# bee-hive/MedGP

Hardware: AMD Instinct MI355X
Metric: per-patient nlml+grad evals/sec at D=24 N=512 (higher is better)
Workload: dtype f64; 1 GPU; config 4 shard: 512 patients/GPU x N=512, D=24, Q=5, R=8, H=1114, LMC-SM + hier-gamma prior, nlml+grad; patients_per_gpu=512, cohort=512, N=512, D=24, Q=5, R=8, H=1114, parallelism=patient-sharded x1 (no collective)

## Files before the change

medgp_amd/csrc/call_plan.h:

```cpp
#pragma once
#include <algorithm>
#include <cstddef>
#include <vector>

#ifndef MEDGP_HD
#if defined(__HIPCC__) || defined(__HIP__)
#define MEDGP_HD __host__ __device__
#else
#define MEDGP_HD
#endif
#endif

#define LA_SLICE 4
MEDGP_HD inline int la_slice_len(int k) { return k < 32 ? LA_SLICE : (k < 44 ? LA_SLICE + 1 : LA_SLICE + 2); }

struct PlanRules {
    int Q = 0, D = 0;
    int num_cu = 256;
    int max_batch = 0;
    size_t mem_budget = (size_t)64 << 30;
    size_t screen_budget = (size_t)2 << 30;
    long long screen_work = 32768;
    int screen_lanes = 2;
    int no_classes = 0;
// ... 25 lines not shown
    int row0 = 0;
    size_t mat0 = 0, vec0 = 0, tab0 = 0, la_part0 = 0, la_small0 = 0;
};

inline int tri(int n) { return n * (n + 1) / 2; }
inline int blocks64(int n) { return (std::max(n, 1) + 63) / 64; }
inline int size_bucket(int nb) { int j = 0; while ((1 << j) < nb) j++; return j; }
inline long long wg_cost(int nb) { return (long long)nb * nb * (nb + 17); }

struct WgradGrid { bool ragged; int nbp, wg_tiles; int grid; };
inline WgradGrid wgrad_grid(const int *entry_n, int nbatch, int nt64) {
    WgradGrid g{false, nbatch, tri(nt64), 0};
    for (int bb = 1; bb < nbatch; bb++) g.ragged = g.ragged || blocks64(entry_n[bb]) != blocks64(entry_n[0]);
    if (g.ragged && nbatch < 64) g.nbp = nbatch | 1;
    g.grid = std::max(8 * ((nbatch + 7) / 8), g.nbp) * g.wg_tiles;
    return g;
}

struct SlabGeom { int R, C; size_t stride; };
inline SlabGeom slab_geom(int ld, int Q, int D) {
    SlabGeom g{ld / 16 + D, ld / 64 + D, 0};
    g.stride = (size_t)3 * Q * g.R * g.C;
    return g;
}

inline void layout_plan(const PlanRules &r, const int *en, int nbatch, bool with_u, BatchPlan &P) {
    P.order.resize(nbatch); P.inv.resize(nbatch); P.en.resize(nbatch);
    P.cls.clear();
    P.with_u = with_u;
    int mx = 0;
    for (int b = 0; b < nbatch; b++) { P.order[b] = b; mx = std::max(mx, en[b]); }
    const bool classes = !r.no_classes;
    if (classes) std::stable_sort(P.order.begin(), P.order.end(), [&](int a, int b) { return blocks64(en[a]) > blocks64(en[b]); });
    P.identity = true;
    for (int i = 0; i < nbatch; i++) { P.inv[P.order[i]] = i; P.en[i] = en[P.order[i]]; P.identity = P.identity && P.order[i] == i; }
    const size_t Q = r.Q, bpe = with_u ? 16 : 8;
    size_t om = 0, ov = 0, ot = 0, os = 0, wave_bytes = 0;
    int wave = 0;
    P.need_mat = P.need_vec = P.need_tab = P.need_slab = 0;
    for (int i = 0; i < nbatch;) {
        SizeClass k;
        k.b0 = i;
        const int bk = size_bucket(blocks64(P.en[i]));
        k.nbmax = classes ? blocks64(P.en[i]) : blocks64(mx);
        k.ld = 64 * k.nbmax;
        const size_t per = bpe * (size_t)k.ld * k.ld;
// ... 133 lines not shown
```

medgp_amd/csrc/kernels_core.h:

```cpp
#pragma once
#include "medgp_dev.h"

#define PREP_CHUNK 2048
#define PREP_BCHUNK 256
__device__ __forceinline__ double prep_w(const MedgpDev &L, const double *th, int q) {
    if (L.kidx == 7) return 2.0 * L.pi * exp(th[L.D + L.Q * L.D * L.R + q]);
    if (L.kidx == 8) return 2.0 * L.pi * exp(th[1 + L.Q + q]);
    return 0.0;
}
__global__ void __launch_bounds__(256) k_prep(MedgpDev L, const double *__restrict__ theta, int min_n) {
    const int b = blockIdx.x, tid = threadIdx.x, nt = blockDim.x;
    const int slot = L.bslot[b];
    const int n = L.pn[slot];
    const double *th = theta + (size_t)(L.tpos ? L.tpos[b] : (L.bpos ? L.bpos[b] : b)) * L.H;
    double *hyp = L.hyp + (size_t)b * L.hyp_stride;
    double *sig2 = hyp, *B = hyp + hyp_off_B(L), *w = hyp + hyp_off_w(L), *c = hyp + hyp_off_c(L);
    const int Q = L.Q, D = L.D, R = L.R;
    const double pi = L.pi;
    const int ntab = (Q * L.ldn + PREP_CHUNK - 1) / PREP_CHUNK;
    if ((int)blockIdx.y > ntab) {
        if (theta == nullptr || L.kidx != 7) return;
        const int idx = ((int)blockIdx.y - ntab - 1) * PREP_BCHUNK + tid;
        if (idx >= Q * D * D) return;
        const double *A = th + D, *lk = th + D + Q * (D * R + 2);
// ... 83 lines not shown
    const int ld = L.ldn;
    const double *hyp = L.hyp + (size_t)b * L.hyp_stride;
    const double *cs = L.cs + (size_t)b * L.Q * ld, *sn = L.sn + (size_t)b * L.Q * ld;
    const double *t = L.pt + (size_t)slot * L.pld;
    const int *meta = L.pmeta + (size_t)slot * L.pld;
    double *K = L.Kmat + (size_t)b * ld * ld;
    for (int idx = threadIdx.x; idx < np * np; idx += blockDim.x) {
        int i = idx / np, j = idx - i * np;
        if (j > i) continue;
        double v;
        if (i < n && j < n) {
            v = cov_elem(L, hyp, cs, sn, t, meta, i, j);
            if (i == j) {
                double lik = hyp[meta[i]];
                v += lik;
                for (int r = 0; r < count; r++) v += lik;
            }
        } else v = (i == j) ? 1.0 : 0.0;
        K[(size_t)i * ld + j] = v;
    }
    __syncthreads();
}

__global__ void __launch_bounds__(256) k_slabsum(MedgpDev L) {
    __shared__ int s_roff[MEDGP_MAX_D + 1], s_coff[MEDGP_MAX_D + 1], s_seg[MEDGP_MAX_D + 1];
    const int b = blockIdx.x, tid = threadIdx.x, nt = blockDim.x;
    if (L.status[b] < 0) return;
    const int Q = L.Q, D = L.D;
    const int slot = L.bslot[b];
    for (int i = tid; i <= D; i += nt) {
        s_roff[i] = L.proff[(size_t)slot * (D + 1) + i];
        s_coff[i] = L.pcoff[(size_t)slot * (D + 1) + i];
        s_seg[i] = L.pseg[(size_t)slot * (D + 1) + i];
    }
    __syncthreads();
    const int *roff = s_roff, *coff = s_coff, *seg = s_seg;
    const double *slab = L.slab + (size_t)b * L.slab_stride;
    const int nbins = D * (D + 1) / 2;
    const int idx = blockIdx.y * nt + tid;
    if (idx >= 3 * Q * nbins) return;
    const int pq = idx / nbins;
    int d, e;
    tile_decode(idx - pq * nbins, d, e);
    const double *sl = slab + (size_t)pq * L.slab_R * L.slab_C;
    double s = 0.0;
    for (int rs = roff[d]; rs < roff[d + 1]; rs++) {
        const int It = (seg[d] / 16 + (rs - roff[d])) / 4;
        for (int cs = coff[e]; cs < coff[e + 1]; cs++) {
            const int Jt = seg[e] / 64 + (cs - coff[e]);
            if (Jt <= It) s += sl[(size_t)rs * L.slab_C + cs];
        }
    }
    const int pl = pq / Q, q = pq - pl * Q;
    double *dst = (pl == 0 ? L.S : (pl == 1 ? L.SM : L.SV)) + (size_t)b * Q * D * D;
    dst[(size_t)q * D * D + d * D + e] = s;
}

__device__ inline void prior_apply(const MedgpPrior &p, double hv, double pi, bool want_grad, double &lp_sum, double &g) {
    if (!p.flag) return;
    if (p.type == 0) { if (want_grad) g = 0.0; return; }
    double lp, dlp;
    if (p.type == 1) {
        lp = -1.0 * (hv - p.p0) * (hv - p.p0) / (2.0 * p.p1);
        lp = lp - log(2 * pi * p.p1) / 2.0;
        dlp = -1.0 * (hv - p.p0) / p.p1;
    } else if (p.type == 2) {
        lp = (-1.0 * fabs(hv - p.p0) / p.p1) - (double)p.lg2b;
        if (hv == p.p0) dlp = 0.0;
        else dlp = -1.0 * ((hv > p.p0) ? 1.0 : -1.0) / p.p1;
    } else return;
    lp_sum += lp;
    if (want_grad) g -= p.is_exp ? hv * dlp : dlp;
}

__device__ inline double sym_get(const double *S, int D, int d, int e) { return d >= e ? S[d * D + e] : S[e * D + d]; }

__global__ void __launch_bounds__(256) k_epilogue(MedgpDev L, const double *__restrict__ theta, int flag_grad, int from_slab,
                                                  double *__restrict__ nlml_out, double *__restrict__ grad_out,
                                                  int *__restrict__ status_out, int loo_objective = 0) {
    __shared__ double red2[MEDGP_EPI_PARTS][256];
    constexpr int EPI_S_MAX = 4096, EPI_A_MAX = 1280;
    __shared__ double s_S[EPI_S_MAX], s_A[EPI_A_MAX];
    const int b = blockIdx.x, tid = threadIdx.x, nt = blockDim.x;
    const int H = L.H, Q = L.Q, D = L.D, R = L.R, ld = L.ldn;
    const int part = blockIdx.y, nparts = gridDim.y;
    const int nchunk = min(MEDGP_EPI_PARTS, (H + 255) / 256), hchunk = (H + nchunk - 1) / nchunk;
    const int cpp = (nchunk + nparts - 1) / nparts, ch0 = part * cpp, ch1 = min(nchunk, ch0 + cpp);
    const int h0 = ch0 * hchunk, h1 = min(H, ch1 * hchunk);
    const int hA0 = L.kidx == 7 ? D : H, hA1 = L.kidx == 7 ? D + Q * D * R : H, hMV1 = L.kidx == 7 ? D + Q * (D * R + 2) : H;
    const bool own_A = h0 < hA1 && h1 > hA0, own_muv = h0 < hMV1 && h1 > hA1;
    const bool lds_sa = flag_grad && L.kidx == 7 && own_A && Q * D * D <= EPI_S_MAX && Q * D * R <= EPI_A_MAX;
    const int st = L.status[b];
    const int pos = L.bpos ? L.bpos[b] : b;
    double *g = grad_out ? grad_out + (size_t)pos * H : nullptr;
    if (tid == 0 && part == 0 && status_out) status_out[pos] = st;
    if (st < 0) {
        if (tid == 0 && part == 0 && loo_objective != 2) nlml_out[pos] = __builtin_nan("");
        if (flag_grad && g) for (int h = h0 + tid; h < h1; h += nt) g[h] = __builtin_nan("");
        return;
    }
    const int slot = L.bslot[b], n = L.pn[slot];
    const double *th = theta + (size_t)(L.tpos ? L.tpos[b] : pos) * H;
    const double *hyp = L.hyp + (size_t)b * L.hyp_stride;
    const double *B = hyp + hyp_off_B(L);
    const double *S = L.S + (size_t)b * Q * D * D, *SM = L.SM + (size_t)b * Q * D * D, *SV = L.SV + (size_t)b * Q * D * D;
    const int *seg = L.pseg + (size_t)slot * (D + 1);
    const double *Wd = from_slab ? L.wdiag + (size_t)b * ld : L.Kmat + (size_t)b * ld * ld;
    const size_t wds = from_slab ? 1 : (size_t)ld + 1;
    if (lds_sa) {
        for (int i = tid; i < Q * D * D; i += nt) s_S[i] = S[i];
        for (int i = tid; i < Q * D * R; i += nt) s_A[i] = th[D + i];
        __syncthreads();
    }
    __shared__ double smuv[64];
    const bool par_muv = flag_grad && L.kidx == 7 && own_muv && 2 * Q <= 64;
    if (par_muv) {
        const int nbins = D * (D + 1) / 2, lane = tid & 63, nwave = nt >> 6;
        for (int w2 = tid >> 6; w2 < 2 * Q; w2 += nwave) {
            const int q = (w2 < Q) ? w2 : w2 - Q;
            const double *X = ((w2 < Q) ? SM : SV) + (size_t)q * D * D, *Bq = B + (size_t)q * D * D;
            double sacc = 0.0;
            int d, e;
            tile_decode(lane, d, e);
            for (int idx = lane; idx < nbins; idx += 64) {
                sacc += ((d == e) ? 1.0 : 2.0) * Bq[d * D + e] * X[d * D + e];
                e += 64;
                while (e > d) { e -= d + 1; d++; }
            }
            for (int off = 32; off > 0; off >>= 1) sacc += __shfl_xor(sacc, off);
            if (lane == 0) smuv[w2] = sacc;
        }
        __syncthreads();
    }
    __shared__ double s_sig[MEDGP_MAX_D];
    const bool par_sig = flag_grad && L.kidx == 7 && h0 < D;
    if (par_sig) {
        const int lane = tid & 63, nwave = nt >> 6, dhi = min(D, h1);
        for (int d = h0 + (tid >> 6); d < dhi; d += nwave) {
            double sacc = 0.0;
            for (int i = seg[d] + lane; i < seg[d + 1]; i += 64) sacc += Wd[(size_t)i * wds];
            for (int off = 32; off > 0; off >>= 1) sacc += __shfl_xor(sacc, off);
            if (lane == 0) s_sig[d] = sacc;
        }
        __syncthreads();
    }
    const int pslot = slot >= L.max_slots ? slot - L.max_slots : slot;
    const MedgpPrior *pr = (loo_objective != 2 && L.prior_on[pslot]) ? L.prior + (size_t)pslot * H : nullptr;
    double lp_part = 0.0;
  for (int ch = ch0; ch < ch1; ch++) {
    double lp_local = 0.0;
    const int hc1 = min(H, (ch + 1) * hchunk);
    for (int h = ch * hchunk + tid; h < hc1; h += nt) {
        double gv = 0.0, hv;
        if (L.kidx == 7) {
            if (h < D) {
                hv = exp(th[h]);
                if (flag_grad) gv = (hv * hv) * s_sig[h];
            } else {
                int hc = h - D;
                if (hc < Q * D * R) {
                    hv = th[h];
                    if (flag_grad) {
                        int q = hc / (D * R), rem = hc - q * D * R, d = rem / R, r = rem - d * R;
                        double s = 0.0;
                        if (lds_sa) {
                            const double *A = s_A + q * D * R, *Sq = s_S + q * D * D;
                            for (int e = 0; e < D; e++) s += sym_get(Sq, D, d, e) * A[e * R + r];
                        } else {
                            const double *A = th + D + (size_t)q * D * R;
                            const double *Sq = S + (size_t)q * D * D;
                            int e = 0;
                            for (; e + 8 <= D; e += 8) {
                                double sv[8], av[8];
#pragma unroll
                                for (int u = 0; u < 8; u++) {
                                    const int ee = e + u, ix = (d >= ee) ? d * D + ee : ee * D + d;
                                    sv[u] = Sq[ix];
                                    av[u] = A[ee * R + r];
                                }
#pragma unroll
                                for (int u = 0; u < 8; u++) s += sv[u] * av[u];
                            }
                            for (; e < D; e++) s += sym_get(Sq, D, d, e) * A[e * R + r];
                        }
                        gv = s;
                    }
                } else if (hc < Q * (D * R + 2)) {
                    hv = exp(th[h]);
                    if (flag_grad) {
                        bool is_mu = hc < Q * (D * R + 1);
                        int q = is_mu ? hc - Q * D * R : hc - Q * (D * R + 1);
                        if (par_muv) gv = 0.5 * smuv[is_mu ? q : Q + q];
                        else {
                            const double *X = (is_mu ? SM : SV) + (size_t)q * D * D, *Bq = B + (size_t)q * D * D;
                            double s = 0.0;
                            for (int d = 0; d < D; d++)
                                for (int e = 0; e <= d; e++) s += ((d == e) ? 1.0 : 2.0) * Bq[d * D + e] * X[d * D + e];
                            gv = 0.5 * s;
                        }
                    }
                } else {
                    hv = exp(th[h]);
                    if (flag_grad) {
                        int kk = hc - Q * (D * R + 2), q = kk / D, d = kk - q * D;
                        gv = 0.5 * hv * S[(size_t)q * D * D + d * D + d];
                    }
                }
            }
        } else if (L.kidx == 8) {
            hv = exp(th[h]);
            if (flag_grad) {
                if (h == 0) {
                    double s = 0.0;
                    for (int i = 0; i < n; i++) s += hv * hv * Wd[(size_t)i * wds];
                    gv = s;
                } else {
                    int hc = h - 1, mode = hc / Q, q = hc - mode * Q;
                    const double *X = mode == 0 ? S : (mode == 1 ? SM : SV);
                    gv = 0.5 * B[q] * X[q];
                }
            }
        } else {
            hv = exp(th[h]);
            if (flag_grad) {
                if (h == 0) {
                    double s = 0.0;
                    for (int i = 0; i < n; i++) s += hv * hv * Wd[(size_t)i * wds];
                    gv = s;
                } else if (h == 1) gv = -0.5 * B[0] * SV[0];
                else gv = B[0] * S[0];
            }
        }
        if (pr) prior_apply(pr[h], hv, L.pi, flag_grad != 0, lp_local, gv);
        if (flag_grad && g) g[h] = gv;
    }
    red2[ch - ch0][tid] = lp_local;
  }
    {
        const int nc = ch1 - ch0;
        __syncthreads();
        for (int off = 128; off > 0; off >>= 1) {
            if (tid < off)
                for (int c2 = 0; c2 < nc; c2++) red2[c2][tid] += red2[c2][tid + off];
            __syncthreads();
        }
        if (tid == 0)
            for (int c2 = 0; c2 < nc; c2++) {
                if (nparts > 1) __hip_atomic_store(&L.epi_lp[(size_t)b * MEDGP_EPI_PARTS + ch0 + c2], red2[c2][0], __ATOMIC_RELAXED, __HIP_MEMORY_SCOPE_AGENT);
                lp_part += red2[c2][0];
            }
    }
    if (tid == 0) {
        double lp = lp_part;
        if (nparts > 1) {
            __threadfence();
            const int ticket = __hip_atomic_fetch_add(&L.epi_ticket[b], 1, __ATOMIC_ACQ_REL, __HIP_MEMORY_SCOPE_AGENT);
            if (ticket != nparts - 1) return;
            __threadfence();
            lp = 0.0;
            for (int c2 = 0; c2 < nchunk; c2++)
                lp += __hip_atomic_load(&L.epi_lp[(size_t)b * MEDGP_EPI_PARTS + c2], __ATOMIC_RELAXED, __HIP_MEMORY_SCOPE_AGENT);
            __hip_atomic_store(&L.epi_ticket[b], 0, __ATOMIC_RELAXED, __HIP_MEMORY_SCOPE_AGENT);
        }
        double logdet = L.scal[b * 4 + 0], quad = L.scal[b * 4 + 1];
        double nlml = quad / 2.0 + logdet + n * log(2. * L.pi) / 2.0;
        if (loo_objective) nlml = L.scal[b * 4 + 2];
        if (loo_objective != 2) nlml_out[pos] = nlml - lp;
    }
}
```

medgp_amd/csrc/medgp_capi.hip:

```cpp
#include "../../include/medgp_hip.h"
#include "medgp_dev.h"
#include "call_plan.h"
#include "kernels_core.h"
#include "kernels_v0.h"
#include "kernels_cholinv.h"
#include "kernels_cholinv_la.h"
#include "kernels_assemble.h"
#include "kernels_wgrad.h"
#include "kernels_io.h"
#include "kernels_cohort.h"
#include "kernels_gmm.h"
#include "kernels_posterior.h"
#include "kernels_posterior_joint.h"
#include "kernels_forecast.h"
#include "kernels_trend.h"
#include "kernels_components.h"
#include "kernels_functional.h"
#include "kernels_functional_joint.h"
#include "kernels_loo.h"
#include "kernels_loo_grad.h"
#include "kernels_forecast_grad.h"
#include "kernels_lgo_grad.h"
#include "kernels_fisher.h"
#include "kernels_hess.h"
// ... 77 lines not shown
    double alloc_s = 0.0;
    long long alloc_calls = 0;
    int *d_bpos = nullptr;
    int *d_tpos = nullptr;
    bool tpos_on = false;
    double *d_screen_theta = nullptr;
    size_t screen_theta_cap = 0;
    bool last_has_inverse = false;
    char *h_stage = nullptr, *d_stage = nullptr;
    size_t stage_cap = 0;
    hipEvent_t ev_stage = nullptr;
    bool stage_pending = false;
    char *h_bounce = nullptr;
    size_t bounce_cap = 0;
    int *d_one_slot = nullptr;
    DevBuf buf[BUF_COUNT];
    size_t posterior_budget = (size_t)2 << 30;
    bool profiling = false;
    int profile_only = -1;
    int wgrad_deep = -1;
    int la_park = 256;
    int la_park_maxbatch = 8;
    int dbg_fail = 0;
    int class_streams = kAuxStreams;
    hipStream_t aux[kAuxStreams] = {nullptr, nullptr, nullptr, nullptr};
    hipEvent_t ev_fork = nullptr, ev_join[kAuxStreams] = {nullptr, nullptr, nullptr, nullptr};
    hipStream_t s_screen1 = nullptr;
    hipEvent_t ev_fork1 = nullptr, ev_screen0 = nullptr;
    char *h_screen_tab = nullptr;
    size_t screen_tab_cap = 0;
    std::vector<EvPair> events;
    std::vector<hipEvent_t> ev_pool;
    double prof_ms[KID_COUNT] = {0};
    int64_t prof_n[KID_COUNT] = {0};
    std::string err;
};

namespace {

int fail(medgp_ctx *c, int code, const char *fmt, ...) {
    char buf[512];
    va_list ap;
    va_start(ap, fmt);
    vsnprintf(buf, sizeof buf, fmt, ap);
    va_end(ap);
    if (c) c->err = buf; else g_create_error = buf;
// ... 327 lines not shown
    int rc;
    if ((rc = arena_ensure(c, AR_LA_PART, need_part * sizeof(double), 0, false, nullptr))) return rc;
    if ((rc = arena_ensure(c, AR_LA_SMALL, need_small * sizeof(double), 0, false, nullptr))) return rc;
    double *pp = (double *)c->arena[AR_LA_PART].base + part0, *ps = (double *)c->arena[AR_LA_SMALL].base + small0;
    args.clear();
    for (const LaNeed &e : v) {
        const LaLayout Y = la_layout(e, with_u);
        LaArgs A{};
        A.nbmax = e.nbmax; A.maxslice = Y.maxslice; A.rows = Y.rows;
        A.ring = 1;
        A.nbatch = e.count;
        A.part = pp;
        A.ybuf = ps + Y.ybuf; A.xk2 = ps + Y.xk2; A.pnx = ps + Y.pnx; A.pnx2 = ps + Y.pnx2;
        A.dterm = ps + Y.dterm; A.dsum = ps + Y.dsum; A.dpart = ps + Y.dpart;
        A.flag = (int *)(ps + Y.flag);
        args.push_back(A);
        pp += Y.part_doubles; ps += Y.small_doubles;
    }
    return MEDGP_OK;
}

int run_pipeline_one(medgp_ctx *c, hipStream_t stream, const MedgpDev &L, int nbatch, int nt64, const double *theta_dev,
                     int flag_grad, bool need_inverse, int min_n, double *nlml_dev, double *grad_dev, int32_t *status_dev,
                     bool store_ukk, const int *entry_n, int route, const LaArgs *la_in) {
    const WgradGrid wg = wgrad_grid(entry_n, nbatch, nt64);
    const bool ragged = wg.ragged;
    { Launcher l(c, KID_PREP, stream); hipLaunchKernelGGL(k_prep, dim3(nbatch, 1 + (L.Q * L.ldn + PREP_CHUNK - 1) / PREP_CHUNK + ((theta_dev && L.kidx == 7) ? (L.Q * L.D * L.D + PREP_BCHUNK - 1) / PREP_BCHUNK : 0)), dim3(256), 0, stream, L, theta_dev, min_n); }
    auto launch_assemble = [&]() {
        Launcher l(c, KID_ASSEMBLE, stream);
        const dim3 tg(tri(nt64), nbatch), tb(256);
        if (c->rules.use_v0 || !with_q16(L.Q, [&](auto q, auto q0) { hipLaunchKernelGGL((k_assemble_t<decltype(q)::value, decltype(q0)::value>), tg, tb, 0, stream, L); }))
            hipLaunchKernelGGL(k_assemble_v0, tg, tb, 0, stream, L);
    };
    const bool inv = flag_grad || need_inverse;
    const int want_mode = inv ? 1 : (store_ukk ? 2 : 0);
    const bool multi_cu = route == ROUTE_LA;
    if (multi_cu) {
        bool any_small = false;
        for (int bb = 0; bb < nbatch; bb++) any_small = any_small || entry_n[bb] <= 64;
        {
            const LaArgs la = *la_in;
            launch_assemble();
            if (any_small) { Launcher l(c, KID_CHOLINV, stream); hipLaunchKernelGGL((k_cholinv<8, 4, 1>), dim3(nbatch), dim3(512), 0, stream, L, want_mode); }
            const int nbx = ragged ? (nbatch | 1) : nbatch;
            { Launcher l(c, KID_LA_AUX, stream); hipLaunchKernelGGL(k_la_prologue, dim3(nbx, 1 + nt64), dim3(LA_THREADS), 0, stream, L, la, want_mode); }
            auto step_counts = [&](int k, int *nF, int *nLrows, int *nsl) {
                const int nMF = std::max(nt64 - (k + 2), 0), nUF = (want_mode & 1) ? k + 1 : 0, nUL = (want_mode & 1) ? k : 0;
// ... 27 lines not shown
    }
    int from_slab = 0;
#ifdef MEDGP_STAMPS
    if (getenv("MEDGP_DBG_NOWGRAD")) { HIPCHK(c, hipGetLastError()); return MEDGP_OK; }
#endif
    if (flag_grad) {
        const int wg_tiles = wg.wg_tiles, nbp = wg.nbp;
        const dim3 tg(wg.grid), tb(WG_THREADS);
        Launcher lw(c, KID_WGRAD, stream);
        const int pf = c->wgrad_deep >= 0 ? c->wgrad_deep : ((long)nbatch * wg_tiles <= 16L * c->rules.num_cu ? 2 : 1);
        from_slab = !c->rules.use_v0 && with_q16(L.Q, [&](auto q, auto q0) {
            constexpr int QQ = decltype(q)::value, Q0 = decltype(q0)::value;
            if (pf >= 2) hipLaunchKernelGGL((k_wgrad<QQ, Q0, 2>), tg, tb, 0, stream, L, nbatch, wg_tiles, nbp);
            else hipLaunchKernelGGL((k_wgrad<QQ, Q0, 1>), tg, tb, 0, stream, L, nbatch, wg_tiles, nbp);
        });
        if (!from_slab) lw.kid = -1;
        lw.finish();
        if (!from_slab) {
            { Launcher l(c, KID_LAUUM, stream); hipLaunchKernelGGL(k_lauum_v0, dim3(tri(nt64), nbatch), dim3(256), 0, stream, L); }
            const int nbins = L.Q * tri(L.D);
            { Launcher l(c, KID_GRADBINS, stream); hipLaunchKernelGGL(k_gradbins_v0, dim3((nbins + 255) / 256, nbatch), dim3(256), 0, stream, L); }
        }
    }
    if (flag_grad && from_slab) {
        const int nbins3 = 3 * L.Q * tri(L.D);
        Launcher l(c, KID_EPILOGUE, stream);
        hipLaunchKernelGGL(k_slabsum, dim3(nbatch, (nbins3 + 255) / 256), dim3(256), 0, stream, L);
    }
    if (nlml_dev) {
        Launcher l(c, KID_EPILOGUE, stream);
        const int nparts = (2 * nbatch >= c->rules.num_cu) ? 1 : std::min(MEDGP_EPI_PARTS, (L.H + 255) / 256);
        hipLaunchKernelGGL(k_epilogue, dim3(nbatch, nparts), dim3(256), 0, stream, L, theta_dev, flag_grad, from_slab, nlml_dev, grad_dev, (int *)status_dev);
    }
    HIPCHK(c, hipGetLastError());
    return MEDGP_OK;
}


int run_pipeline(medgp_ctx *c, const double *theta_dev, int flag_grad, bool need_inverse, int min_n,
                 double *nlml_dev, double *grad_dev, int32_t *status_dev, bool store_ukk = false, bool persist = false,
                 BatchPlan *Pp = nullptr, hipStream_t st_main = nullptr, int aux0 = 0, int naux = kAuxStreams, hipEvent_t ev_fork_in = nullptr) {
    BatchPlan &P = Pp ? *Pp : c->plan;
    if (!st_main) st_main = c->stream;
    hipEvent_t ev_fork = ev_fork_in ? ev_fork_in : c->ev_fork;
    const bool forms_u = flag_grad || need_inverse || store_ukk;
    if (forms_u && !P.with_u) return fail(c, MEDGP_ERR_ARG, "internal: plan laid out without Linv for a call that forms it");
    if (persist && P.nwaves > 1)
        return fail(c, MEDGP_ERR_CAPACITY, "the call's per-entry matrices exceed the memory budget of %zu GB (MEDGP_MEM_BUDGET_GB) and its outputs need all of them at once: split the call",
                    c->rules.mem_budget >> 30);
    std::vector<LaNeed> las;
    std::vector<int> la_of;
    const PlanNeeds nd = plan_needs(c->rules, P, las, la_of);
    { int rc = ensure_arena(c, P.mat0 + nd.mat, P.with_u ? P.mat0 + nd.mat : 0, P.vec0 + nd.vec, P.tab0 + nd.tab, nd.slab); if (rc) return rc; }
    c->last_has_inverse = (flag_grad || need_inverse) && P.nwaves == 1;
// ... 2 lines not shown
        size_t i0 = 0, i1;
        while (i0 < P.cls.size() && P.cls[i0].wave != w) i0++;
        i1 = i0;
        while (i1 < P.cls.size() && P.cls[i1].wave == w) i1++;
        std::vector<LaNeed> wl;
        std::vector<int> wl_of(P.cls.size(), -1);
        for (size_t i = i0; i < i1; i++) if (la_of[i] >= 0) { wl_of[i] = (int)wl.size(); wl.push_back(las[la_of[i]]); }
        std::vector<LaArgs> wa;
        if (!wl.empty()) { int rc = ensure_la(c, wl, P.with_u, wa, P.la_part0, P.la_small0); if (rc) return rc; }
        const bool fork = i1 - i0 > 1 && nstr > 0 && c->aux[aux0];
        if (fork) HIPCHK(c, hipEventRecord(ev_fork, st_main));
        bool used[kAuxStreams] = {false, false, false, false};
        for (size_t i = i0; i < i1; i++) {
            const SizeClass &k = P.cls[i];
            hipStream_t st = st_main;
            int ai = -1;
            if (fork && i > i0) {
                ai = aux0 + (int)((i - i0 - 1) % nstr);
                st = c->aux[ai];
                if (!used[ai]) { HIPCHK(c, hipStreamWaitEvent(st, ev_fork, 0)); used[ai] = true; }
            }
            const MedgpDev V = class_view(c, P, k);
            int rc = run_pipeline_one(c, st, V, k.count, k.nbmax, theta_dev, flag_grad, need_inverse, min_n, nlml_dev, grad_dev, status_dev, store_ukk,
                                      P.en.data() + k.b0, k.route, wl_of[i] >= 0 ? &wa[wl_of[i]] : nullptr);
            if (rc) return rc;
        }
        if (fork)
            for (int ai = aux0; ai < aux0 + nstr; ai++)
                if (used[ai]) {
                    HIPCHK(c, hipEventRecord(c->ev_join[ai], c->aux[ai]));
                    HIPCHK(c, hipStreamWaitEvent(st_main, c->ev_join[ai], 0));
                }
    }
    return MEDGP_OK;
}

int check_call(medgp_ctx *c, int nbatch, const int32_t *slots) {
    if (c->max_slots == 0) return fail(c, MEDGP_ERR_CAPACITY, "call medgp_reserve first");
    if (nbatch < 1 || nbatch > c->rules.max_batch) return fail(c, MEDGP_ERR_CAPACITY, "nbatch %d outside [1, %d]", nbatch, c->rules.max_batch);
    for (int b = 0; b < nbatch; b++)
        if (slots[b] < 0 || slots[b] >= c->max_slots || c->h_n[slots[b]] < 0) return fail(c, MEDGP_ERR_ARG, "slots[%d] = %d is not a resident patient", b, slots[b]);
    return MEDGP_OK;
}

int check_points(medgp_ctx *c, int nbatch, const int64_t *offsets, const int32_t *meta2, const float *t2, const float *mean, const float *var,
                 const char *outs = "mean / var") {
    if (offsets[0] != 0) return fail(c, MEDGP_ERR_ARG, "offsets[0] = %lld, expected 0", (long long)offsets[0]);
// ... 84 lines not shown
    if (kernel_index == MEDGP_KERNEL_SM) { D = 1; R = 0; }
    int nc = num_cov(kernel_index, Q, D, R);
    if (nc < 0) return fail(nullptr, MEDGP_ERR_ARG, "unsupported kernel_index %d (supported: 0 SE, 7 LMC-SM, 8 SM)", kernel_index);
    if (Q < 1 || D < 1 || R < 0) return fail(nullptr, MEDGP_ERR_ARG, "bad Q/D/R = %d/%d/%d", Q, D, R);
    if (D > MEDGP_MAX_D) return fail(nullptr, MEDGP_ERR_ARG, "D = %d exceeds the supported %d outputs", D, MEDGP_MAX_D);
    int ndev = medgp_device_count();
    if (ndev <= 0) return fail(nullptr, MEDGP_ERR_NODEVICE, "no HIP device visible; libmedgp_hip has no CPU fallback");
    if (device < 0 || device >= ndev) return fail(nullptr, MEDGP_ERR_ARG, "device %d outside [0, %d)", device, ndev);
    medgp_ctx *c = new medgp_ctx();
    c->device = device;
    c->kidx = kernel_index; c->rules.Q = Q; c->rules.D = D; c->R = R;
    c->nlik = (kernel_index == MEDGP_KERNEL_LMC_SM) ? D : 1;
    c->H = c->nlik + nc;
    if (hipSetDevice(device) != hipSuccess || hipStreamCreateWithFlags(&c->own_stream, hipStreamNonBlocking) != hipSuccess) {
        delete c;
        return fail(nullptr, MEDGP_ERR_HIP, "cannot initialise device %d", device);
    }
    c->stream = c->own_stream;
    { const char *e = getenv("MEDGP_CHOLINV_NW"); c->rules.cholinv_nw = e ? atoi(e) : 0; }
    { const char *e = getenv("MEDGP_LA_PARK"); if (e) c->la_park = atoi(e); }
    { const char *e = getenv("MEDGP_LA_PARK_MAXBATCH"); if (e) c->la_park_maxbatch = atoi(e); }
    { const char *e = getenv("MEDGP_MULTI_CU"); c->rules.force_mc = e ? atoi(e) : 0; }
    { const char *e = getenv("MEDGP_CLASS_STREAMS"); if (e) c->class_streams = std::max(0, std::min(kAuxStreams, atoi(e))); }
    { const char *e = getenv("MEDGP_NO_CLASSES"); c->rules.no_classes = e ? atoi(e) : 0; }
    { const char *e = getenv("MEDGP_WGRAD_DEEP"); c->wgrad_deep = e ? std::max(1, atoi(e)) : -1; }
    { const char *e = getenv("MEDGP_DEBUG_FAIL_ATTEMPTS"); c->dbg_fail = e ? atoi(e) : 0; }
    { const char *e = getenv("MEDGP_V0"); c->rules.use_v0 = e && e[0] == '1'; }
    { const char *e = getenv("MEDGP_MEM_BUDGET_GB"); if (e && atof(e) > 0) c->rules.mem_budget = (size_t)(atof(e) * 1073741824.0); }
    { const char *e = getenv("MEDGP_SCREEN_LANES"); if (e && atoi(e) >= 1) c->rules.screen_lanes = std::min(2, atoi(e)); }
    { const char *e = getenv("MEDGP_SCREEN_WORK"); if (e && atoll(e) > 0) c->rules.screen_work = atoll(e); }
    { const char *e = getenv("MEDGP_SCREEN_BUDGET_GB"); if (e && atof(e) > 0) c->rules.screen_budget = (size_t)(atof(e) * 1073741824.0); }
    { const char *e = getenv("MEDGP_POSTERIOR_BUDGET_GB"); if (e && atof(e) > 0) c->posterior_budget = (size_t)(atof(e) * 1073741824.0); }
    for (int i = 0; i < kAuxStreams; i++) {
        (void)hipStreamCreateWithFlags(&c->aux[i], hipStreamNonBlocking);
        (void)hipEventCreateWithFlags(&c->ev_join[i], hipEventDisableTiming);
    }
    (void)hipEventCreateWithFlags(&c->ev_fork, hipEventDisableTiming);
    (void)hipStreamCreateWithFlags(&c->s_screen1, hipStreamNonBlocking);
    for (hipEvent_t *e : {&c->ev_fork1, &c->ev_screen0}) (void)hipEventCreateWithFlags(e, hipEventDisableTiming);
    { hipDeviceProp_t pr; if (hipGetDeviceProperties(&pr, device) == hipSuccess) c->rules.num_cu = pr.multiProcessorCount; }
    *out = c;
    return MEDGP_OK;
}

void medgp_destroy(medgp_ctx *c) {
    if (!c) return;
// ... 628 lines not shown
    HIPCHK(c, hipMemcpyAsync(&st, E.status, sizeof(int), hipMemcpyDeviceToHost, c->stream));
    HIPCHK(c, hipStreamSynchronize(c->stream));
    if (st < 0) return fail(c, MEDGP_ERR_ARG, "batch entry %d failed (status %d); no factor available", b, st);
    if (linv && eff < S && !c->h_perm_identity[slot]) {
        const int shadow = slot + S;
        HIPCHK(c, hipMemcpyAsync(c->d_one_slot, &shadow, sizeof(int), hipMemcpyHostToDevice, c->stream));
        MedgpDev V = E;
        V.bslot = c->d_one_slot;
        V.bpos = nullptr;
        const bool prof = c->profiling;
        c->profiling = false;
        BatchPlan P1;
        std::vector<LaNeed> las;
        std::vector<int> la_of;
        std::vector<LaArgs> la;
        layout_plan(c->rules, &n, 1, true, P1);
        choose_routes(c->rules, P1, las, la_of);
        if (!las.empty()) {
            las[0].ld = ld;
            int rcl = ensure_la(c, las, true, la);
            if (rcl) return rcl;
        }
        const SizeClass &k1 = P1.cls[0];
        int rc = run_pipeline_one(c, c->stream, V, 1, k1.nbmax, nullptr, 0, true, 1, nullptr, nullptr, nullptr, false, &n, k1.route, la.empty() ? nullptr : &la[0]);
        c->profiling = prof;
        if (rc) return rc;
        HIPCHK(c, hipMemcpyAsync((int *)E.bslot, c->d_one_slot, sizeof(int), hipMemcpyDeviceToDevice, c->stream));
        HIPCHK(c, hipMemcpyAsync(&st, E.status, sizeof(int), hipMemcpyDeviceToHost, c->stream));
        HIPCHK(c, hipStreamSynchronize(c->stream));
        c->h_bslot[b] = eff = shadow;
        if (st < 0) return fail(c, MEDGP_ERR_ARG, "batch entry %d: the factorisation in the caller's order failed (status %d)", b, st);
    }
    const bool caller_order = eff >= S || c->h_perm_identity[slot];
    if (alpha) {
        std::vector<double> ha(n);
        HIPCHK(c, hipMemcpy(ha.data(), E.alpha, sizeof(double) * n, hipMemcpyDeviceToHost));
        for (int i = 0; i < n; i++) alpha[caller_order ? i : perm[i]] = (float)ha[i];
    }
    if (beta) {
        double sc[4];
        HIPCHK(c, hipMemcpy(sc, E.scal, sizeof(sc), hipMemcpyDeviceToHost));
        *beta = (float)sc[1];
    }
    if (linv) {
        const char *hp = nullptr;
        int rc2 = d2h_pinned(c, E.Linv, sizeof(double) * n * ld, &hp);
        if (rc2) return rc2;
// ... 1400 lines not shown
```

Measured before the change: 198,300 evals/s.

## Fuse slab bin summation into the epilogue as a single k_finish kernel

Adds a k_finish kernel that sums slab bins directly into packed triangular LDS planes and then runs the epilogue body. This removes the separate k_slabsum launch and the global S/SM/SV round trip. It also prefetches theta A entries, diagonal W values, B coefficients and prior records into registers before the bin reduction to hide latency, and restructures the slab summation into flattened unrolled loads. The fused path is taken only for LMC kernels with one class and one epilogue part. It costs more LDS per block and a one-block-per-patient grid.

```diff
diff --git a/medgp_amd/csrc/call_plan.h b/medgp_amd/csrc/call_plan.h
--- a/medgp_amd/csrc/call_plan.h
+++ b/medgp_amd/csrc/call_plan.h
@@ -71,6 +71,30 @@
     SlabGeom g{ld / 16 + D, ld / 64 + D, 0};
     g.stride = (size_t)3 * Q * g.R * g.C;
     return g;
+}
+
+#define FIN_POOL 7424
+#define FIN_MAX_D 64
+#define FIN_MAX_A 1280
+struct FinishLayout { int nbins, nchunk, off_a, off_s, off_sm, off_red, total; };
+MEDGP_HD inline FinishLayout finish_layout(int Q, int D, int R, int H) {
+    FinishLayout Y{};
+    Y.nbins = D * (D + 1) / 2;
+    const int c = (H + 255) / 256;
+    Y.nchunk = c < 16 ? c : 16;
+    const int planes2 = 2 * Q * Y.nbins, red = Y.nchunk * 256;
+    Y.off_a = 0;
+    Y.off_s = Q * D * R;
+    Y.off_sm = Y.off_s + Q * Y.nbins;
+    Y.off_red = Y.off_sm;
+    Y.total = Y.off_sm + (planes2 > red ? planes2 : red);
+    return Y;
+}
+inline bool finish_fused(bool enabled, int kidx, int Q, int D, int R, int H, bool flag_grad, bool has_nlml, bool from_slab, int nparts, int nclasses) {
+    if (!enabled || !flag_grad || !has_nlml || !from_slab || kidx != 7) return false;
+    if (nparts != 1 || nclasses != 1) return false;
+    if (Q < 1 || Q > 8 || D < 1 || D > FIN_MAX_D || R < 1 || Q * D * R > FIN_MAX_A) return false;
+    return finish_layout(Q, D, R, H).total <= FIN_POOL;
 }
 
 inline void layout_plan(const PlanRules &r, const int *en, int nbatch, bool with_u, BatchPlan &P) {
diff --git a/medgp_amd/csrc/kernels_core.h b/medgp_amd/csrc/kernels_core.h
--- a/medgp_amd/csrc/kernels_core.h
+++ b/medgp_amd/csrc/kernels_core.h
@@ -1,5 +1,6 @@
 #pragma once
 #include "medgp_dev.h"
+#include "call_plan.h"
 
 #define PREP_CHUNK 2048
 #define PREP_BCHUNK 256
@@ -129,6 +130,48 @@
     __syncthreads();
 }
 
+__device__ inline void tile_decode_small(int x, int &I, int &J) {
+    int i = (int)((sqrtf(8.0f * (float)x + 1.0f) - 1.0f) * 0.5f);
+    while ((i + 1) * (i + 2) / 2 <= x) i++;
+    while (i * (i + 1) / 2 > x) i--;
+    I = i;
+    J = x - i * (i + 1) / 2;
+}
+
+#define SLAB_P 6
+struct SlabBin { const double *p; int nc, total, it0, jt0; };
+__device__ __forceinline__ SlabBin slab_bin(const MedgpDev &L, const int *roff, const int *coff, const int *seg, const double *slab, int nbins, int idx) {
+    const int pq = idx / nbins;
+    int d, e;
+    tile_decode_small(idx - pq * nbins, d, e);
+    SlabBin b;
+    b.nc = coff[e + 1] - coff[e];
+    b.total = (roff[d + 1] - roff[d]) * b.nc;
+    b.it0 = seg[d] / 16;
+    b.jt0 = seg[e] / 64;
+    b.p = slab + (size_t)pq * L.slab_R * L.slab_C + (size_t)roff[d] * L.slab_C + coff[e];
+    return b;
+}
+__device__ __forceinline__ unsigned slab_bin_load(const SlabBin &b, int slab_C, int k0, double (&v)[SLAB_P]) {
+    int r = 0, cc = k0;
+    if (k0 > 0) { r = k0 / b.nc; cc = k0 - r * b.nc; }
+    unsigned ok = 0;
+#pragma unroll
+    for (int u = 0; u < SLAB_P; u++) {
+        const int It = (b.it0 + r) / 4, Jt = b.jt0 + cc;
+        const bool in = k0 + u < b.total && Jt <= It;
+        v[u] = in ? b.p[(size_t)r * slab_C + cc] : 0.0;
+        ok |= in ? 1u << u : 0u;
+        if (++cc >= b.nc) { cc = 0; r++; }
+    }
+    return ok;
+}
+__device__ __forceinline__ void slab_bin_add(double &s, const double (&v)[SLAB_P], unsigned ok) {
+#pragma unroll
+    for (int u = 0; u < SLAB_P; u++)
+        if (ok >> u & 1) s += v[u];
+}
+
 __global__ void __launch_bounds__(256) k_slabsum(MedgpDev L) {
     __shared__ int s_roff[MEDGP_MAX_D + 1], s_coff[MEDGP_MAX_D + 1], s_seg[MEDGP_MAX_D + 1];
     const int b = blockIdx.x, tid = threadIdx.x, nt = blockDim.x;
@@ -141,24 +184,19 @@
         s_seg[i] = L.pseg[(size_t)slot * (D + 1) + i];
     }
     __syncthreads();
-    const int *roff = s_roff, *coff = s_coff, *seg = s_seg;
     const double *slab = L.slab + (size_t)b * L.slab_stride;
     const int nbins = D * (D + 1) / 2;
     const int idx = blockIdx.y * nt + tid;
     if (idx >= 3 * Q * nbins) return;
-    const int pq = idx / nbins;
+    const SlabBin bn = slab_bin(L, s_roff, s_coff, s_seg, slab, nbins, idx);
+    double s = 0.0, v[SLAB_P];
+    for (int k = 0; k < bn.total; k += SLAB_P) {
+        const unsigned ok = slab_bin_load(bn, L.slab_C, k, v);
+        slab_bin_add(s, v, ok);
+    }
+    const int pq = idx / nbins, pl = pq / Q, q = pq - pl * Q;
     int d, e;
-    tile_decode(idx - pq * nbins, d, e);
-    const double *sl = slab + (size_t)pq * L.slab_R * L.slab_C;
-    double s = 0.0;
-    for (int rs = roff[d]; rs < roff[d + 1]; rs++) {
-        const int It = (seg[d] / 16 + (rs - roff[d])) / 4;
-        for (int cs = coff[e]; cs < coff[e + 1]; cs++) {
-            const int Jt = seg[e] / 64 + (cs - coff[e]);
-            if (Jt <= It) s += sl[(size_t)rs * L.slab_C + cs];
-        }
-    }
-    const int pl = pq / Q, q = pq - pl * Q;
+    tile_decode_small(idx - pq * nbins, d, e);
     double *dst = (pl == 0 ? L.S : (pl == 1 ? L.SM : L.SV)) + (size_t)b * Q * D * D;
     dst[(size_t)q * D * D + d * D + e] = s;
 }
@@ -182,21 +220,34 @@
 
 __device__ inline double sym_get(const double *S, int D, int d, int e) { return d >= e ? S[d * D + e] : S[e * D + d]; }
 
-__global__ void __launch_bounds__(256) k_epilogue(MedgpDev L, const double *__restrict__ theta, int flag_grad, int from_slab,
-                                                  double *__restrict__ nlml_out, double *__restrict__ grad_out,
-                                                  int *__restrict__ status_out, int loo_objective = 0) {
-    __shared__ double red2[MEDGP_EPI_PARTS][256];
+struct EpiLds {
+    double (*red2)[256];
+    double *s_S, *s_A;
+    double *smuv, *s_sig;
+    double *planes;
+    const int *seg;
+};
+#define FIN_WPF 8
+#define FIN_BPF 8
+struct EpiNoStage { __device__ void tables() const {} __device__ void bins() const {} };
+
+template <bool FUSED, class Stage>
+__device__ __forceinline__ void epilogue_body(const MedgpDev &L, const double *__restrict__ theta, int flag_grad, int from_slab,
+                                              double *__restrict__ nlml_out, double *__restrict__ grad_out, int *__restrict__ status_out,
+                                              int loo_objective, const EpiLds &M, const Stage &stage) {
     constexpr int EPI_S_MAX = 4096, EPI_A_MAX = 1280;
-    __shared__ double s_S[EPI_S_MAX], s_A[EPI_A_MAX];
+    double (*red2)[256] = M.red2;
+    double *s_S = M.s_S, *s_A = M.s_A, *smuv = M.smuv, *s_sig = M.s_sig;
     const int b = blockIdx.x, tid = threadIdx.x, nt = blockDim.x;
     const int H = L.H, Q = L.Q, D = L.D, R = L.R, ld = L.ldn;
-    const int part = blockIdx.y, nparts = gridDim.y;
+    const int part = FUSED ? 0 : blockIdx.y, nparts = FUSED ? 1 : gridDim.y;
     const int nchunk = min(MEDGP_EPI_PARTS, (H + 255) / 256), hchunk = (H + nchunk - 1) / nchunk;
     const int cpp = (nchunk + nparts - 1) / nparts, ch0 = part * cpp, ch1 = min(nchunk, ch0 + cpp);
     const int h0 = ch0 * hchunk, h1 = min(H, ch1 * hchunk);
-    const int hA0 = L.kidx == 7 ? D : H, hA1 = L.kidx == 7 ? D + Q * D * R : H, hMV1 = L.kidx == 7 ? D + Q * (D * R + 2) : H;
+    const bool lmc = FUSED || L.kidx == 7;
+    const int hA0 = lmc ? D : H, hA1 = lmc ? D + Q * D * R : H, hMV1 = lmc ? D + Q * (D * R + 2) : H;
     const bool own_A = h0 < hA1 && h1 > hA0, own_muv = h0 < hMV1 && h1 > hA1;
-    const bool lds_sa = flag_grad && L.kidx == 7 && own_A && Q * D * D <= EPI_S_MAX && Q * D * R <= EPI_A_MAX;
+    const bool lds_sa = FUSED || (flag_grad && lmc && own_A && Q * D * D <= EPI_S_MAX && Q * D * R <= EPI_A_MAX);
     const int st = L.status[b];
     const int pos = L.bpos ? L.bpos[b] : b;
     double *g = grad_out ? grad_out + (size_t)pos * H : nullptr;
@@ -210,27 +261,73 @@
     const double *th = theta + (size_t)(L.tpos ? L.tpos[b] : pos) * H;
     const double *hyp = L.hyp + (size_t)b * L.hyp_stride;
     const double *B = hyp + hyp_off_B(L);
-    const double *S = L.S + (size_t)b * Q * D * D, *SM = L.SM + (size_t)b * Q * D * D, *SV = L.SV + (size_t)b * Q * D * D;
-    const int *seg = L.pseg + (size_t)slot * (D + 1);
+    const int nbins = D * (D + 1) / 2, pst = FUSED ? nbins : D * D;
+    auto sx = [&](int d, int e) { return FUSED ? d * (d + 1) / 2 + e : d * D + e; };
+    const double *S = FUSED ? M.planes : L.S + (size_t)b * Q * D * D;
+    const double *SM = FUSED ? M.planes + Q * nbins : L.SM + (size_t)b * Q * D * D;
+    const double *SV = FUSED ? M.planes + 2 * Q * nbins : L.SV + (size_t)b * Q * D * D;
     const double *Wd = from_slab ? L.wdiag + (size_t)b * ld : L.Kmat + (size_t)b * ld * ld;
     const size_t wds = from_slab ? 1 : (size_t)ld + 1;
-    if (lds_sa) {
+    const int pslot = slot >= L.max_slots ? slot - L.max_slots : slot;
+    const MedgpPrior *pr = (loo_objective != 2 && L.prior_on[pslot]) ? L.prior + (size_t)pslot * H : nullptr;
+    const int *seg = FUSED ? M.seg : L.pseg + (size_t)slot * (D + 1);
+    double pf_a[FUSED ? FIN_MAX_A / 256 : 1], pf_w[FUSED ? FIN_WPF : 1], pf_b[FUSED ? FIN_BPF : 1];
+    MedgpPrior pf_p{};
+    if constexpr (FUSED) {
+        stage.tables();
+        const int lane = tid & 63, wv = tid >> 6;
+#pragma unroll
+        for (int k = 0; k < FIN_MAX_A / 256; k++) { const int i = tid + 256 * k; pf_a[k] = i < Q * D * R ? th[D + i] : 0.0; }
+#pragma unroll
+        for (int u = 0; u < FIN_WPF; u++) {
+            const int d = wv + 4 * u;
+            pf_w[u] = (d < D && seg[d] + lane < seg[d + 1]) ? Wd[(size_t)(seg[d] + lane) * wds] : 0.0;
+        }
+        {
+            const double *Bq = B + (size_t)(wv < Q ? wv : wv - Q) * D * D;
+            int d, e;
+            tile_decode_small(lane, d, e);
+#pragma unroll
+            for (int u = 0; u < FIN_BPF; u++) {
+                pf_b[u] = (wv < 2 * Q && lane + 64 * u < nbins) ? Bq[d * D + e] : 0.0;
+                e += 64;
+                while (e > d) { e -= d + 1; d++; }
+            }
+        }
+        if (pr && tid < H) pf_p = pr[tid];
+        stage.bins();
+#pragma unroll
+        for (int k = 0; k < FIN_MAX_A / 256; k++) { const int i = tid + 256 * k; if (i < Q * D * R) s_A[i] = pf_a[k]; }
+        __syncthreads();
+    } else if (lds_sa) {
         for (int i = tid; i < Q * D * D; i += nt) s_S[i] = S[i];
         for (int i = tid; i < Q * D * R; i += nt) s_A[i] = th[D + i];
         __syncthreads();
     }
-    __shared__ double smuv[64];
-    const bool par_muv = flag_grad && L.kidx == 7 && own_muv && 2 * Q <= 64;
+    const bool par_muv = FUSED || (flag_grad && lmc && own_muv && 2 * Q <= 64);
     if (par_muv) {
-        const int nbins = D * (D + 1) / 2, lane = tid & 63, nwave = nt >> 6;
+        const int lane = tid & 63, nwave = nt >> 6;
         for (int w2 = tid >> 6; w2 < 2 * Q; w2 += nwave) {
             const int q = (w2 < Q) ? w2 : w2 - Q;
-            const double *X = ((w2 < Q) ? SM : SV) + (size_t)q * D * D, *Bq = B + (size_t)q * D * D;
+            const double *X = ((w2 < Q) ? SM : SV) + (size_t)q * pst, *Bq = B + (size_t)q * D * D;
             double sacc = 0.0;
             int d, e;
             tile_decode(lane, d, e);
-            for (int idx = lane; idx < nbins; idx += 64) {
-                sacc += ((d == e) ? 1.0 : 2.0) * Bq[d * D + e] * X[d * D + e];
+            int idx = lane;
+            if constexpr (FUSED) {
+                if (w2 == (tid >> 6)) {
+#pragma unroll
+                    for (int u = 0; u < FIN_BPF; u++)
+                        if (idx < nbins) {
+                            sacc += ((d == e) ? 1.0 : 2.0) * pf_b[u] * X[sx(d, e)];
+                            e += 64;
+                            while (e > d) { e -= d + 1; d++; }
+                            idx += 64;
+                        }
+                }
+            }
+            for (; idx < nbins; idx += 64) {
+                sacc += ((d == e) ? 1.0 : 2.0) * Bq[d * D + e] * X[sx(d, e)];
                 e += 64;
                 while (e > d) { e -= d + 1; d++; }
             }
@@ -239,27 +336,33 @@
         }
         __syncthreads();
     }
-    __shared__ double s_sig[MEDGP_MAX_D];
-    const bool par_sig = flag_grad && L.kidx == 7 && h0 < D;
+    const bool par_sig = FUSED || (flag_grad && lmc && h0 < D);
     if (par_sig) {
         const int lane = tid & 63, nwave = nt >> 6, dhi = min(D, h1);
-        for (int d = h0 + (tid >> 6); d < dhi; d += nwave) {
+        auto sig_one = [&](int d, bool have, double w0) {
             double sacc = 0.0;
-            for (int i = seg[d] + lane; i < seg[d + 1]; i += 64) sacc += Wd[(size_t)i * wds];
+            int i = seg[d] + lane;
+            if (have && i < seg[d + 1]) { sacc += w0; i += 64; }
+            for (; i < seg[d + 1]; i += 64) sacc += Wd[(size_t)i * wds];
             for (int off = 32; off > 0; off >>= 1) sacc += __shfl_xor(sacc, off);
             if (lane == 0) s_sig[d] = sacc;
-        }
+        };
+        int d = h0 + (tid >> 6);
+        if constexpr (FUSED) {
+#pragma unroll
+            for (int u = 0; u < FIN_WPF; u++, d += nwave)
+                if (d < dhi) sig_one(d, true, pf_w[u]);
+        }
+        for (; d < dhi; d += nwave) sig_one(d, false, 0.0);
         __syncthreads();
     }
-    const int pslot = slot >= L.max_slots ? slot - L.max_slots : slot;
-    const MedgpPrior *pr = (loo_objective != 2 && L.prior_on[pslot]) ? L.prior + (size_t)pslot * H : nullptr;
     double lp_part = 0.0;
   for (int ch = ch0; ch < ch1; ch++) {
     double lp_local = 0.0;
     const int hc1 = min(H, (ch + 1) * hchunk);
     for (int h = ch * hchunk + tid; h < hc1; h += nt) {
         double gv = 0.0, hv;
-        if (L.kidx == 7) {
+        if (lmc) {
             if (h < D) {
                 hv = exp(th[h]);
                 if (flag_grad) gv = (hv * hv) * s_sig[h];
@@ -271,8 +374,8 @@
                         int q = hc / (D * R), rem = hc - q * D * R, d = rem / R, r = rem - d * R;
                         double s = 0.0;
                         if (lds_sa) {
-                            const double *A = s_A + q * D * R, *Sq = s_S + q * D * D;
-                            for (int e = 0; e < D; e++) s += sym_get(Sq, D, d, e) * A[e * R + r];
+                            const double *A = s_A + q * D * R, *Sq = s_S + q * pst;
+                            for (int e = 0; e < D; e++) s += (d >= e ? Sq[sx(d, e)] : Sq[sx(e, d)]) * A[e * R + r];
                         } else {
                             const double *A = th + D + (size_t)q * D * R;
                             const double *Sq = S + (size_t)q * D * D;
@@ -310,7 +413,7 @@
                     hv = exp(th[h]);
                     if (flag_grad) {
                         int kk = hc - Q * (D * R + 2), q = kk / D, d = kk - q * D;
-                        gv = 0.5 * hv * S[(size_t)q * D * D + d * D + d];
+                        gv = 0.5 * hv * S[(size_t)q * pst + sx(d, d)];
                     }
                 }
             }
@@ -338,7 +441,10 @@
                 else gv = B[0] * S[0];
             }
         }
-        if (pr) prior_apply(pr[h], hv, L.pi, flag_grad != 0, lp_local, gv);
+        if (pr) {
+            if (FUSED && h == tid) prior_apply(pf_p, hv, L.pi, flag_grad != 0, lp_local, gv);
+            else prior_apply(pr[h], hv, L.pi, flag_grad != 0, lp_local, gv);
+        }
         if (flag_grad && g) g[h] = gv;
     }
     red2[ch - ch0][tid] = lp_local;
@@ -375,3 +481,71 @@
         if (loo_objective != 2) nlml_out[pos] = nlml - lp;
     }
 }
+
+__global__ void __launch_bounds__(256) k_epilogue(MedgpDev L, const double *__restrict__ theta, int flag_grad, int from_slab,
+                                                  double *__restrict__ nlml_out, double *__restrict__ grad_out,
+                                                  int *__restrict__ status_out, int loo_objective = 0) {
+    __shared__ double red2[MEDGP_EPI_PARTS][256];
+    __shared__ double s_S[4096], s_A[1280];
+    __shared__ double smuv[64];
+    __shared__ double s_sig[MEDGP_MAX_D];
+    const EpiLds M{red2, s_S, s_A, smuv, s_sig, nullptr, nullptr};
+    epilogue_body<false>(L, theta, flag_grad, from_slab, nlml_out, grad_out, status_out, loo_objective, M, EpiNoStage{});
+}
+
+#define SLAB_G 6
+struct FinishStage {
+    const MedgpDev &L;
+    int *roff, *coff, *seg;
+    double *planes;
+    __device__ void tables() const {
+        const int tid = threadIdx.x, D = L.D, slot = L.bslot[blockIdx.x];
+        for (int i = tid; i <= D; i += 256) {
+            roff[i] = L.proff[(size_t)slot * (D + 1) + i];
+            coff[i] = L.pcoff[(size_t)slot * (D + 1) + i];
+            seg[i] = L.pseg[(size_t)slot * (D + 1) + i];
+        }
+        __syncthreads();
+    }
+    __device__ void bins() const {
+        const int tid = threadIdx.x, nbins = L.D * (L.D + 1) / 2, nb3 = 3 * L.Q * nbins;
+        const double *slab = L.slab + (size_t)blockIdx.x * L.slab_stride;
+        for (int i0 = tid; i0 < nb3; i0 += SLAB_G * 256) {
+            SlabBin bn[SLAB_G];
+            double v[SLAB_G][SLAB_P];
+            unsigned ok[SLAB_G];
+#pragma unroll
+            for (int j = 0; j < SLAB_G; j++) {
+                const int idx = i0 + 256 * j;
+                if (idx < nb3) bn[j] = slab_bin(L, roff, coff, seg, slab, nbins, idx);
+                else bn[j] = SlabBin{slab, 0, 0, 0, 0};
+            }
+#pragma unroll
+            for (int j = 0; j < SLAB_G; j++) ok[j] = slab_bin_load(bn[j], L.slab_C, 0, v[j]);
+#pragma unroll
+            for (int j = 0; j < SLAB_G; j++) {
+                double s = 0.0;
+                slab_bin_add(s, v[j], ok[j]);
+                for (int k = SLAB_P; k < bn[j].total; k += SLAB_P) {
+                    double w[SLAB_P];
+                    const unsigned okw = slab_bin_load(bn[j], L.slab_C, k, w);
+                    slab_bin_add(s, w, okw);
+                }
+                if (i0 + 256 * j < nb3) planes[i0 + 256 * j] = s;
+            }
+        }
+    }
+};
+
+__global__ void __launch_bounds__(256) k_finish(MedgpDev L, const double *__restrict__ theta, double *__restrict__ nlml_out,
+                                                double *__restrict__ grad_out, int *__restrict__ status_out, int loo_objective) {
+    __shared__ double pool[FIN_POOL];
+    __shared__ double smuv[64], s_sig[FIN_MAX_D];
+    __shared__ int s_roff[FIN_MAX_D + 1], s_coff[FIN_MAX_D + 1], s_seg[FIN_MAX_D + 1];
+    static_assert(sizeof(double) * (FIN_POOL + 64 + FIN_MAX_D) + sizeof(int) * 3 * (FIN_MAX_D + 1) <= 64 * 1024, "k_finish: static LDS");
+    static_assert(FIN_MAX_A % 256 == 0 && FIN_MAX_D <= MEDGP_MAX_D, "k_finish: prefetch registers / tables");
+    const FinishLayout Y = finish_layout(L.Q, L.D, L.R, L.H);
+    const EpiLds M{(double (*)[256])(pool + Y.off_red), pool + Y.off_s, pool + Y.off_a, smuv, s_sig, pool + Y.off_s, s_seg};
+    const FinishStage stage{L, s_roff, s_coff, s_seg, pool + Y.off_s};
+    epilogue_body<true>(L, theta, 1, 1, nlml_out, grad_out, status_out, loo_objective, M, stage);
+}
diff --git a/medgp_amd/csrc/medgp_capi.hip b/medgp_amd/csrc/medgp_capi.hip
--- a/medgp_amd/csrc/medgp_capi.hip
+++ b/medgp_amd/csrc/medgp_capi.hip
@@ -123,6 +123,7 @@
     int la_park = 256;
     int la_park_maxbatch = 8;
     int dbg_fail = 0;
+    bool finish_fused = true;
     int class_streams = kAuxStreams;
     hipStream_t aux[kAuxStreams] = {nullptr, nullptr, nullptr, nullptr};
     hipEvent_t ev_fork = nullptr, ev_join[kAuxStreams] = {nullptr, nullptr, nullptr, nullptr};
@@ -496,7 +497,7 @@
 
 int run_pipeline_one(medgp_ctx *c, hipStream_t stream, const MedgpDev &L, int nbatch, int nt64, const double *theta_dev,
                      int flag_grad, bool need_inverse, int min_n, double *nlml_dev, double *grad_dev, int32_t *status_dev,
-                     bool store_ukk, const int *entry_n, int route, const LaArgs *la_in) {
+                     bool store_ukk, const int *entry_n, int route, const LaArgs *la_in, int nclasses) {
     const WgradGrid wg = wgrad_grid(entry_n, nbatch, nt64);
     const bool ragged = wg.ragged;
     { Launcher l(c, KID_PREP, stream); hipLaunchKernelGGL(k_prep, dim3(nbatch, 1 + (L.Q * L.ldn + PREP_CHUNK - 1) / PREP_CHUNK + ((theta_dev && L.kidx == 7) ? (L.Q * L.D * L.D + PREP_BCHUNK - 1) / PREP_BCHUNK : 0)), dim3(256), 0, stream, L, theta_dev, min_n); }
@@ -570,6 +571,13 @@
             { Launcher l(c, KID_GRADBINS, stream); hipLaunchKernelGGL(k_gradbins_v0, dim3((nbins + 255) / 256, nbatch), dim3(256), 0, stream, L); }
         }
     }
+    const int nparts = (2 * nbatch >= c->rules.num_cu) ? 1 : std::min(MEDGP_EPI_PARTS, (L.H + 255) / 256);
+    if (finish_fused(c->finish_fused, L.kidx, L.Q, L.D, L.R, L.H, flag_grad != 0, nlml_dev != nullptr, from_slab != 0, nparts, nclasses)) {
+        Launcher l(c, KID_EPILOGUE, stream);
+        hipLaunchKernelGGL(k_finish, dim3(nbatch), dim3(256), 0, stream, L, theta_dev, nlml_dev, grad_dev, (int *)status_dev, 0);
+        HIPCHK(c, hipGetLastError());
+        return MEDGP_OK;
+    }
     if (flag_grad && from_slab) {
         const int nbins3 = 3 * L.Q * tri(L.D);
         Launcher l(c, KID_EPILOGUE, stream);
@@ -577,7 +585,6 @@
     }
     if (nlml_dev) {
         Launcher l(c, KID_EPILOGUE, stream);
-        const int nparts = (2 * nbatch >= c->rules.num_cu) ? 1 : std::min(MEDGP_EPI_PARTS, (L.H + 255) / 256);
         hipLaunchKernelGGL(k_epilogue, dim3(nbatch, nparts), dim3(256), 0, stream, L, theta_dev, flag_grad, from_slab, nlml_dev, grad_dev, (int *)status_dev);
     }
     HIPCHK(c, hipGetLastError());
@@ -626,7 +633,7 @@
             }
             const MedgpDev V = class_view(c, P, k);
             int rc = run_pipeline_one(c, st, V, k.count, k.nbmax, theta_dev, flag_grad, need_inverse, min_n, nlml_dev, grad_dev, status_dev, store_ukk,
-                                      P.en.data() + k.b0, k.route, wl_of[i] >= 0 ? &wa[wl_of[i]] : nullptr);
+                                      P.en.data() + k.b0, k.route, wl_of[i] >= 0 ? &wa[wl_of[i]] : nullptr, (int)P.cls.size());
             if (rc) return rc;
         }
         if (fork)
@@ -757,6 +764,7 @@
     { const char *e = getenv("MEDGP_LA_PARK_MAXBATCH"); if (e) c->la_park_maxbatch = atoi(e); }
     { const char *e = getenv("MEDGP_MULTI_CU"); c->rules.force_mc = e ? atoi(e) : 0; }
     { const char *e = getenv("MEDGP_CLASS_STREAMS"); if (e) c->class_streams = std::max(0, std::min(kAuxStreams, atoi(e))); }
+    { const char *e = getenv("MEDGP_FINISH_FUSED"); if (e) c->finish_fused = atoi(e) != 0; }
     { const char *e = getenv("MEDGP_NO_CLASSES"); c->rules.no_classes = e ? atoi(e) : 0; }
     { const char *e = getenv("MEDGP_WGRAD_DEEP"); c->wgrad_deep = e ? std::max(1, atoi(e)) : -1; }
     { const char *e = getenv("MEDGP_DEBUG_FAIL_ATTEMPTS"); c->dbg_fail = e ? atoi(e) : 0; }
@@ -1431,7 +1439,7 @@
             if (rcl) return rcl;
         }
         const SizeClass &k1 = P1.cls[0];
-        int rc = run_pipeline_one(c, c->stream, V, 1, k1.nbmax, nullptr, 0, true, 1, nullptr, nullptr, nullptr, false, &n, k1.route, la.empty() ? nullptr : &la[0]);
+        int rc = run_pipeline_one(c, c->stream, V, 1, k1.nbmax, nullptr, 0, true, 1, nullptr, nullptr, nullptr, false, &n, k1.route, la.empty() ? nullptr : &la[0], 1);
         c->profiling = prof;
         if (rc) return rc;
         HIPCHK(c, hipMemcpyAsync((int *)E.bslot, c->d_one_slot, sizeof(int), hipMemcpyDeviceToDevice, c->stream));
```

Result: no change. 199,600 evals/s, median of 3 (+0.6%).
